# zpaq/zpaq

Hardware: AMD Instinct MI355X
Metric: compress MB/s + bit-identical ratio, -m5 over 1024x1 MiB blocks (higher is better)
Workload: dtype int32

## Files before the change

### zpaq_amd/csrc/device/pipe_kernel.h

```cpp
#pragma once
#ifndef ZPQ_LANE_VM
#define ZPQ_LANE_VM 1
#endif
#include "spec_kernel.h"

namespace zpq {

typedef __attribute__((address_space(1))) short g_i16;
typedef __attribute__((address_space(1))) unsigned short g_u16;

#ifdef ZPQ_TRACE
struct PipeTraceScope {
  unsigned long long* rec;
  __device__ __forceinline__ PipeTraceScope(const PipeArgs& a, int kernel) : rec(nullptr) {
    if (a.trace && threadIdx.x == 0) {
      rec = a.trace + 4ull * ((unsigned long long)a.trace_base + blockIdx.x);
      unsigned hw, xcc;
      asm volatile("s_getreg_b32 %0, hwreg(HW_REG_HW_ID)" : "=s"(hw));
      asm volatile("s_getreg_b32 %0, hwreg(HW_REG_XCC_ID)" : "=s"(xcc));
      rec[0] = ((unsigned long long)(unsigned)kernel << 56) | ((unsigned long long)((unsigned)a.step & 0xFFFFFFu) << 32) |
               (unsigned long long)(blockIdx.x + a.wg0);
      rec[1] = ((unsigned long long)xcc << 32) | hw;
      rec[2] = __builtin_amdgcn_s_memrealtime();
    }
// ... 1807 lines not shown
    unsigned byte = L.byte_at(0);
    uint2 w = L.bh(ri, 0);
    uint4 vj = L.p(J, 0);
    s = pipe_bh_get(w, 0);
    w0 = (int)tab[(2u * s) * G + lane]; w1 = (int)tab[(2u * s + 1u) * G + lane];
    for (unsigned k = 0; k < L.nb; ++k) {
      const unsigned kn = L.next(k);
      const unsigned byten = L.byte_at(kn);
      const uint2 wn = L.bh(ri, kn);
      const uint4 vjn = L.p(J, kn);
      do_byte(k, byte, w, wn, vj);
      byte = byten; w = wn; vj = vjn;
    }
  }
  if (store_tab)
    for (int e = 0; e < 512; e += 4)
      L.A128((unsigned)c.t0 + 4u * e) = make_uint4(tab[e * G + lane], tab[(e + 1) * G + lane], tab[(e + 2) * G + lane], tab[(e + 3) * G + lane]);
}

template <class Chain>
__device__ __forceinline__ void pipe_isse_body(const PipeArgs& a) {
  constexpr unsigned G = Chain::PIPE_G;
  __shared__ unsigned tab[512 * G];
  __shared__ PipeSquash squash;
  const int lane = threadIdx.x & 63;
  const unsigned ngroups = (a.nblocks + Chain::PIPE_G - 1u) / Chain::PIPE_G;
  const unsigned wg = blockIdx.x + a.wg0;
  const unsigned role = wg / ngroups, g = wg % ngroups;
  static_for<0, Chain::NISSE>([&](auto rc) __attribute__((always_inline)) {
    constexpr int r = decltype(rc)::value;
    if (role != (unsigned)r) return;
    constexpr int I = Chain::ISSE_COMP[r];
    PipeLane<Chain> L;
    L.open(a, g * Chain::PIPE_G + (unsigned)lane, Chain::P_LEVEL[I]);
    if (L.chunk < 0 || !pipe_any(L.nb > 0)) return;
    squash.load(a.tb, lane);
    __syncthreads();
    pipe_isse_unit<Chain, I>(L, tab, squash, lane, true, true);
  });
}

typedef uint4 __attribute__((aligned(4))) pipe_u128a4;
typedef __attribute__((address_space(1))) pipe_u128a4 g_u128a4;

template <int QL>
__device__ __forceinline__ int pipe_group_sum(int v) {
  if constexpr (QL >= 2) v += __builtin_amdgcn_update_dpp(0, v, 0xB1, 0xF, 0xF, true);
  if constexpr (QL >= 4) v += __builtin_amdgcn_update_dpp(0, v, 0x4E, 0xF, 0xF, true);
  if constexpr (QL >= 8) v += __builtin_amdgcn_update_dpp(0, v, 0x141, 0xF, 0xF, true);
  if constexpr (QL >= 16) v += __builtin_amdgcn_update_dpp(0, v, 0x140, 0xF, 0xF, true);
  return v;
}

template <class Chain, int r, class SQ>
__device__ __forceinline__ void pipe_mix_bits_unit(PipeLane<Chain>& L, unsigned q, unsigned B, const SQ& squash) {
  constexpr int I = Chain::MIX_COMP[r], QL = Chain::MIX_QL[r];
  constexpr CompK c = Chain::comp[I];
  constexpr int m = (int)c.a3, J = (int)c.a2, ci = Chain::P_CTX[I];
  constexpr int NQ = (m + 3) / 4, TAIL = m % 4, D = Chain::MIX_DEPTH, HN = D;
  static_assert(NQ <= QL && c.a5 == 255u && c.mask0 >= 255u, "MIX bit lanes need the 8 rows of a byte to be distinct");
  if (!L.nb) return;
  constexpr bool FULL = c.stride >= 4u * (unsigned)QL;
  const bool act = FULL || q < (unsigned)NQ;
  const bool tail = !FULL && TAIL != 0 && q == (unsigned)(NQ - 1);
  const unsigned qoff = 16u * (act ? q : 0u);
  bool have[4];
  int tin[4];
#pragma unroll
  for (int x = 0; x < 4; ++x) {
    const int t = (int)q * 4 + x;
    have[x] = t < m;
    tin[x] = J + (have[x] ? t : 0);
  }
  auto row_of = [&](unsigned hh, unsigned bytev) __attribute__((always_inline)) -> unsigned {
    const unsigned c8 = (1u << B) | (bytev >> (8u - B));
    return (unsigned)c.t0 + 4u * __umul24((hh + c8) & c.mask0, (unsigned)c.stride) + qoff;
  };
  auto input = [&](int x, unsigned kk) __attribute__((always_inline)) -> int {
    return (int)*(const g_i16*)((const g_u8*)&L.p(tin[x], kk) + 2u * B);
  };
  const unsigned last = L.nb - 1u;
  constexpr int W = 2 * D;
  unsigned hx[W], bx[W];
  unsigned rq[W];
  uint4 wq[W];
  int pq[W][4];
  unsigned hr[HN], hh[HN];
  uint4 hw[HN];
  auto near = [&](int sl, unsigned kk) __attribute__((always_inline)) {
    rq[sl] = row_of(hx[sl], bx[sl]);
    wq[sl] = *(g_u128a4*)(L.arena + rq[sl]);
#pragma unroll
    for (int x = 0; x < 4; ++x) pq[sl][x] = input(x, kk);
  };
#pragma unroll
  for (int sl = 0; sl < W; ++sl) {
    const unsigned kk = min((unsigned)sl, last);
    hx[sl] = L.ctx(ci, kk);
    bx[sl] = L.byte_at(kk);
  }
#pragma unroll
  for (int sl = 0; sl < D; ++sl) near(sl, min((unsigned)sl, last));
#pragma unroll
  for (int i = 0; i < HN; ++i) { hr[i] = 0xFFFFFFFFu; hh[i] = hx[0]; hw[i] = make_uint4(0u, 0u, 0u, 0u); }
  for (unsigned kb = 0; pipe_any(kb < L.nb); kb += (unsigned)W) {
#pragma unroll
// ... 31 lines not shown
        else if (act && !tail) *(g_u128a4*)(L.arena + row) = nw;
        if constexpr (TAIL != 0 && !FULL) {
          if (tail) {
            L.A32(row) = nw.x;
            if constexpr (TAIL >= 2) L.A32(row + 4u) = nw.y;
            if constexpr (TAIL >= 3) L.A32(row + 8u) = nw.z;
          }
        }
        if (q == 0) L.put_p16(I, k, B, pr);
      }
#pragma unroll
      for (int i = HN - 1; i > 0; --i) { hr[i] = hr[i - 1]; hh[i] = hh[i - 1]; hw[i] = hw[i - 1]; }
      hr[0] = row; hh[0] = hcur; hw[0] = nw;
      {
        const unsigned kw = min(k + (unsigned)W, last);
        hx[sl] = L.ctx(ci, kw);
        bx[sl] = L.byte_at(kw);
        near((sl + D) % W, min(k + (unsigned)D, last));
      }
    }
  }
}

template <class Chain>
__device__ __forceinline__ void pipe_mix_bits_body(const PipeArgs& a) {
  __shared__ PipeSquash squash;
  const int lane = threadIdx.x & 63;
  const unsigned ngroups = (a.nblocks + Chain::PIPE_G - 1u) / Chain::PIPE_G;
  const unsigned wg = blockIdx.x + a.wg0;
  squash.load(a.tb, lane);
  __syncthreads();
  static_for<0, Chain::NMIXR>([&](auto rc) __attribute__((always_inline)) {
    constexpr int r = decltype(rc)::value;
    constexpr int I = Chain::MIX_COMP[r], QL = Chain::MIX_QL[r], first = Chain::MIX_FIRST[r];
    constexpr int PPW = 64 / QL, BPW = PPW / 8;
    static_assert(QL <= 8 && BPW >= 1 && (int)Chain::PIPE_G % BPW == 0, "MIX bit lanes: a block's 8 positions share a wavefront");
    constexpr int WPG = (int)Chain::PIPE_G / BPW;
    if (wg < (unsigned)first * ngroups || wg >= (unsigned)(first + WPG) * ngroups) return;
    const unsigned wi = wg - (unsigned)first * ngroups;
    const unsigned g = wi / (unsigned)WPG, sub = wi % (unsigned)WPG;
    const unsigned pair = (unsigned)lane / QL, q = (unsigned)lane % QL, B = pair & 7u;
    PipeLane<Chain> L;
    L.open(a, pipe_opaque(g * Chain::PIPE_G + sub * BPW + (pair >> 3)), Chain::P_LEVEL[I]);
    if (L.chunk < 0 || !pipe_any(L.nb > 0)) return;
    pipe_mix_bits_unit<Chain, r>(L, q, B, squash);
  });
}

template <class Chain, int r, int NH, class SQ>
__device__ __forceinline__ void pipe_mix_unit(PipeLane<Chain>& L, unsigned q, unsigned half, const SQ& squash) {
  constexpr int I = Chain::MIX_COMP[r], QL = Chain::MIX_QL[r];
  constexpr CompK c = Chain::comp[I];
  constexpr int m = (int)c.a3, J = (int)c.a2, ci = Chain::P_CTX[I];
  constexpr int NQ = (m + 3) / 4, TAIL = m % 4, NB = 8 / NH;
  static_assert(NQ <= QL, "MIX lane group");
  constexpr bool batch = c.a5 == 255u && c.mask0 >= 255u;
  static_assert(NH == 1 || (NH == 2 && batch), "a byte is split over lane groups only when its 8 rows are distinct");
  if (!L.nb) return;
  constexpr bool FULL = c.stride >= 4u * (unsigned)QL;
  const bool act = FULL || q < (unsigned)NQ;
  const bool tail = !FULL && TAIL != 0 && q == (unsigned)(NQ - 1);
  const unsigned qoff = 16u * (act ? q : 0u);
  bool have[4];
  int tin[4];
#pragma unroll
  for (int x = 0; x < 4; ++x) {
    const int t = (int)q * 4 + x;
    have[x] = t < m;
    tin[x] = J + (have[x] ? t : 0);
  }
  auto c8_of = [&](unsigned bytev, int b) __attribute__((always_inline)) -> unsigned {
    if constexpr (NH == 1) return pipe_c8(bytev, b);
    else return ((half ? 16u : 1u) << b) | ((half ? bytev : bytev >> 4) >> (4 - b));
  };
  auto y_of = [&](unsigned bytev, int b) __attribute__((always_inline)) -> int {
    if constexpr (NH == 1) return pipe_y(bytev, b);
    else return (int)(((half ? bytev : bytev >> 4) >> (3 - b)) & 1u);
  };
  auto row_of = [&](unsigned hh, unsigned bytev, int b) __attribute__((always_inline)) -> unsigned {
    return (unsigned)c.t0 + 4u * __umul24((hh + (c8_of(bytev, b) & c.a5)) & c.mask0, (unsigned)c.stride) + qoff;
  };
  unsigned h = L.ctx(ci, 0), byte = L.byte_at(0);
  const unsigned k1 = L.next(0);
  unsigned h1 = L.ctx(ci, k1), byte1 = L.byte_at(k1);
  auto inputs = [&](int x, unsigned kk) __attribute__((always_inline)) -> uint4 {
    const uint4 v = L.p(tin[x], kk);
    const unsigned mk = have[x] ? 0xFFFFFFFFu : 0u;
    if constexpr (NH == 1) return make_uint4(v.x & mk, v.y & mk, v.z & mk, v.w & mk);
    else return make_uint4((half ? v.z : v.x) & mk, (half ? v.w : v.y) & mk, 0u, 0u);
  };
  uint4 pv[4], pv1[4];
#pragma unroll
  for (int x = 0; x < 4; ++x) { pv[x] = inputs(x, 0); pv1[x] = inputs(x, k1); }
  uint4 w[NB];
  unsigned rowc[NB];
#pragma unroll
  for (int B = 0; B < NB; ++B) rowc[B] = row_of(h, byte, B);
  if constexpr (batch) {
#pragma unroll
    for (int B = 0; B < NB; ++B) w[B] = *(g_u128a4*)(L.arena + rowc[B]);
  }
  for (unsigned k = 0; k < L.nb; ++k) {
    const unsigned k2 = min(k + 2u, L.nb - 1u);
    const unsigned h2 = L.ctx(ci, k2), byte2 = L.byte_at(k2);
    uint4 pv2[4];
#pragma unroll
    for (int x = 0; x < 4; ++x) pv2[x] = inputs(x, k2);
    unsigned rown[NB];
#pragma unroll
    for (int B = 0; B < NB; ++B) rown[B] = row_of(h1, byte1, B);
    const bool same = h1 == h;
    const bool late = !same && (((h1 - h) & c.mask0) < 256u || ((h - h1) & c.mask0) < 256u);
    uint4 wn[NB], nw[NB];
    if constexpr (batch) {
      if (!late) {
#pragma unroll
        for (int B = 0; B < NB; ++B) wn[B] = *(g_u128a4*)(L.arena + rown[B]);
      }
    }
    PipeP8 out;
#pragma unroll
    for (int B = 0; B < NB; ++B) {
      const unsigned row = rowc[B];
      if constexpr (!batch) w[B] = *(g_u128a4*)(L.arena + row);
      const int w0 = (int)w[B].x, w1 = (int)w[B].y, w2 = (int)w[B].z, w3 = (int)w[B].w;
      const int p0 = pipe_p_get(pv[0], B), p1 = pipe_p_get(pv[1], B), p2 = pipe_p_get(pv[2], B), p3 = pipe_p_get(pv[3], B);
      const int dot = __mul24(w0 >> 8, p0) + __mul24(w1 >> 8, p1) + __mul24(w2 >> 8, p2) + __mul24(w3 >> 8, p3);
      const int pr = sp_clamp2k(pipe_group_sum<QL>(dot) >> 8);
      out.set(B, pr);
      const int err = __mul24(y_of(byte, B) * 32767 - squash(pr), (int)c.a4) >> 4;
      nw[B].x = (unsigned)sp_clamp512k(w0 + ((__mul24(err, p0) + (1 << 12)) >> 13));
      nw[B].y = (unsigned)sp_clamp512k(w1 + ((__mul24(err, p1) + (1 << 12)) >> 13));
      nw[B].z = (unsigned)sp_clamp512k(w2 + ((__mul24(err, p2) + (1 << 12)) >> 13));
      nw[B].w = (unsigned)sp_clamp512k(w3 + ((__mul24(err, p3) + (1 << 12)) >> 13));
      if constexpr (FULL) *(g_u128a4*)(L.arena + row) = nw[B];
      else if (act && !tail) *(g_u128a4*)(L.arena + row) = nw[B];
      if constexpr (TAIL != 0 && !FULL) {
        if (tail) {
          L.A32(row) = nw[B].x;
          if constexpr (TAIL >= 2) L.A32(row + 4u) = nw[B].y;
          if constexpr (TAIL >= 3) L.A32(row + 8u) = nw[B].z;
        }
      }
    }
    if (q == 0) {
      if constexpr (NH == 1) L.put_p(I, k, out.get());
      else L.put_p64(I, k, half, make_uint2(out.w[0], out.w[1]));
    }
    if constexpr (batch) {
      if constexpr (NH == 2) {
        if (pipe_any(late)) pipe_stores_done();
      }
      if (late) {
#pragma unroll
        for (int B = 0; B < NB; ++B) wn[B] = *(g_u128a4*)(L.arena + rown[B]);
      }
#pragma unroll
      for (int B = 0; B < NB; ++B) {
        const bool fw = same && rown[B] == rowc[B];
        w[B].x = fw ? nw[B].x : wn[B].x; w[B].y = fw ? nw[B].y : wn[B].y;
        w[B].z = fw ? nw[B].z : wn[B].z; w[B].w = fw ? nw[B].w : wn[B].w;
      }
    }
    h = h1; byte = byte1; h1 = h2; byte1 = byte2;
#pragma unroll
    for (int B = 0; B < NB; ++B) rowc[B] = rown[B];
#pragma unroll
    for (int x = 0; x < 4; ++x) { pv[x] = pv1[x]; pv1[x] = pv2[x]; }
  }
}

struct PipeW3 { unsigned x, y, z; };
typedef __attribute__((address_space(1))) PipeW3 g_w3;

__device__ __forceinline__ int pipe_sext24(unsigned v) { return (int)(v << 8) >> 8; }
__device__ __forceinline__ void pipe_unpack4(const PipeW3& d, int& w0, int& w1, int& w2, int& w3) {
  w0 = pipe_sext24(d.x);
  w1 = pipe_sext24((d.x >> 24) | (d.y << 8));
  w2 = pipe_sext24((d.y >> 16) | (d.z << 16));
  w3 = (int)d.z >> 8;
}
__device__ __forceinline__ PipeW3 pipe_pack4(int w0, int w1, int w2, int w3) {
  PipeW3 d;
  d.x = ((unsigned)w0 & 0xFFFFFFu) | ((unsigned)w1 << 24);
  d.y = (((unsigned)w1 >> 8) & 0xFFFFu) | ((unsigned)w2 << 16);
  d.z = (((unsigned)w2 >> 16) & 0xFFu) | ((unsigned)w3 << 8);
  return d;
}

__device__ __forceinline__ constexpr unsigned pipe_mix_pstride(unsigned m) {
  const unsigned need = 12u * ((m + 3u) / 4u);
  unsigned p = 16u;
  while (p < need) p *= 2u;
  return p;
}

template <class Chain, class = void> struct PipeMixLdsRows { static constexpr int of(int) { return 0; } };
template <class Chain> struct PipeMixLdsRows<Chain, decltype((void)Chain::MIX_LDS_ROWS)> { static constexpr int of(int r) { return Chain::MIX_LDS_ROWS[r]; } };

template <class Chain, int r, int LROWS, int BPW, int NH, class SQ>
__device__ __forceinline__ void pipe_mix_packed_unit(PipeLane<Chain>& L, unsigned q, unsigned half, unsigned bl, unsigned* lds, bool stage, const SQ& squash) {
  constexpr int I = Chain::MIX_COMP[r], QL = Chain::MIX_QL[r];
  constexpr CompK c = Chain::comp[I];
  constexpr int m = (int)c.a3, J = (int)c.a2, ci = Chain::P_CTX[I];
  constexpr int NQ = (m + 3) / 4, NB = 8 / NH;
  constexpr unsigned PS = pipe_mix_pstride((unsigned)m);
  static_assert(NQ <= QL && c.a5 == 255u && c.mask0 >= 255u, "packed MIX rows: the 8 rows of a byte are distinct");
  static_assert(PS <= 4u * c.stride, "a packed row fits the padded row's place");
  static_assert(NH == 1 || NH == 2, "lane groups per block");
  if (!L.nb) return;
  const bool act = q < (unsigned)NQ;
  const unsigned qoff = 12u * (act ? q : 0u);
  bool have[4];
  int tin[4];
#pragma unroll
  for (int x = 0; x < 4; ++x) {
    const int t = (int)q * 4 + x;
    have[x] = t < m;
    tin[x] = J + (have[x] ? t : 0);
  }
  auto c8_of = [&](unsigned bytev, int b) __attribute__((always_inline)) -> unsigned {
// ... 170 lines not shown
```

### zpaq_amd/csrc/device/pipe_persist.h

```cpp
#pragma once
#include "pipe_kernel.h"

#if !defined(ZPQ_EMU)
#ifndef ZPQ_PERSIST_LDS_BYTES
#error "the generated source defines ZPQ_PERSIST_LDS_BYTES before it includes pipe_persist.h"
#endif
namespace zpq { __shared__ __attribute__((aligned(16))) unsigned char persist_lds[ZPQ_PERSIST_LDS_BYTES]; }
#endif

namespace zpq {

struct PipeRO {
  int dt[1024];
  unsigned short dt2k[256];
  PipeSquash squash;
  PipeStretch stretch;
  unsigned char ns[1024];
};

#ifdef ZPQ_EMU
#define ZPQ_PERSIST_LDS(bytes) ((unsigned char*)emu::wg_lds(bytes))
__device__ __forceinline__ unsigned pipe_prog_load(const unsigned* p) { return *(volatile const unsigned*)p; }
__device__ __forceinline__ void pipe_prog_add(unsigned* p) { *(volatile unsigned*)p = *(volatile unsigned*)p + 1u; }
__device__ __forceinline__ void pipe_flag_set(unsigned* p, unsigned v) { *(volatile unsigned*)p = v; }
// ... 198 lines not shown
      }
    } else {
      constexpr int lk = Chain::LIGHT_KIND[role], I = Chain::LIGHT_COMP[role];
      if constexpr (lk == PK_CODER) {
        if constexpr (PipeCoderFast<Chain>::value) pipe_coder_fast<Chain, (PipeAhead<Chain>::value > 0 ? PipeAhead<Chain>::value : 1)>(L, a, (unsigned*)priv, lane, c == 0);
        else pipe_coder<Chain>(L, a, ro.squash);
      } else if (pipe_any(L.nb > 0)) {
        if constexpr (lk == PK_CONS) pipe_cons<Chain, I>(L);
        else if constexpr (lk == PK_CM) {
          if constexpr (pipe_light_lds_words<Chain>(lk, I) != 0u) pipe_cm_lds<Chain, I>(L, (unsigned*)priv, ro.stretch, ro.dt, lane, c == 0);
          else pipe_cm<Chain, I>(L, ro.stretch, ro.dt);
        }
        else if constexpr (lk == PK_MATCH) pipe_match_any<Chain, I>(L, ro.stretch, ro.dt2k);
        else if constexpr (lk == PK_AVG) pipe_avg<Chain, I>(L);
        else if constexpr (lk == PK_MIX2) {
          if constexpr (pipe_light_lds_words<Chain>(lk, I) != 0u) pipe_mix2_lds<Chain, I>(L, (unsigned*)priv, ro.squash, lane, c == 0);
          else pipe_mix2<Chain, I>(L, ro.squash);
        }
        else if constexpr (lk == PK_SSE) pipe_sse<Chain, I>(L, ro.stretch, ro.dt);
        else if constexpr (lk == PK_CM_BITS) pipe_cm_bits<Chain, I>(L, B, ro.stretch, ro.dt);
        else if constexpr (lk == PK_MIX2_BITS) pipe_mix2_bits<Chain, I>(L, B, ro.squash);
        else if constexpr (lk == PK_SSE_BITS) pipe_sse_bits<Chain, I>(L, B, ro.stretch, ro.dt);
      }
    }
    pipe_reconverge();
    pipe_publish<Chain>(prog, unit, lane);
    if (a.trace) { const unsigned long long t = pipe_clock(); t_work += t - t_mark; t_mark = t; }
  }
  if (a.trace && lane == 0) {
    unsigned long long* rec = a.trace + 4ull * ((unsigned long long)g * (unsigned)Chain::PS_NSLOT + (unsigned)SLOT);
    rec[0] = t_wait; rec[1] = t_work; rec[2] = nchunks; rec[3] = ((unsigned long long)kind << 32) | ((unsigned long long)(unsigned)role << 16) | (unsigned)unit;
  }
}

template <class Chain>
__device__ __forceinline__ void pipe_persist_body(const PipeArgs& a) {
  unsigned char* const lds = ZPQ_PERSIST_LDS(Chain::PS_LDS_BYTES);
  PipeRO& ro = *(PipeRO*)lds;
  const int tid = (int)threadIdx.x, lane = tid & 63, wave = tid >> 6;
  for (int i = tid; i < 1024; i += (int)blockDim.x) ro.dt[i] = a.tb->dt[i];
  for (int i = tid; i < 256; i += (int)blockDim.x) ro.dt2k[i] = (unsigned short)a.tb->dt2k[i];
  for (int i = tid; i < 256; i += (int)blockDim.x) ((unsigned*)ro.ns)[i] = ((const unsigned*)a.tb->ns)[i];
  ro.squash.load(a.tb, tid);
  ro.stretch.load(a.tb, tid);
  if (tid == 0 && a.arrive_need) pipe_prog_add(a.ctl + 3);
  __syncthreads();
  const unsigned b = blockIdx.x, nx = a.spread ? a.spread : 1u, W = (unsigned)Chain::PS_WPG;
  const unsigned whole = a.ngroups_here - a.ngroups_here % nx;
  unsigned g, flavour;
  if (b < whole * W) { const unsigned j = b / nx; g = b % nx + nx * (j / W); flavour = j % W; }
  else { const unsigned r = b - whole * W; g = whole + r / W; flavour = r % W; }
  g += a.group0;
  if (g >= a.group0 + a.ngroups_here) return;
  const int slot = (int)flavour * Chain::PS_WAVES + wave;
  if (!pipe_arrived(a, lane)) return;
  static_for<0, Chain::PS_NSLOT>([&](auto sc) __attribute__((always_inline)) {
    constexpr int S = decltype(sc)::value;
    if constexpr (Chain::PS_KIND[S] >= 0) {
      if (slot == S) pipe_persist_unit<Chain, Chain::PS_KIND[S], Chain::PS_ROLE[S]>(a, g, lane, S);
    }
  });
}

}
```

### zpaq_amd/csrc/host/codegen.cpp

```cpp
#include "codegen.hpp"

#include <cstdio>
#include <cstdlib>
#include <cstring>
#include <map>
#include <mutex>
#include <set>
#include <sstream>
#include <algorithm>

namespace zpq {

namespace {

struct Insn { int pc, len, op; };

std::string src_expr(int k, int imm) {
  switch (k) {
    case 0: return "a";
    case 1: return "b";
    case 2: return "c";
    case 3: return "d";
    case 4: return "(unsigned)M[b & MMASK]";
    case 5: return "(unsigned)M[c & MMASK]";
// ... 568 lines not shown
  Memo m;
  m.ok = pipe_layout_compute(plan, opt, m.L, m.why);
  L = m.L; why_not = m.why;
  std::lock_guard<std::mutex> g(mu);
  if (memo.size() > 4096) memo.clear();
  memo[key] = m;
  return m.ok;
}

static bool pipe_layout_compute(const zpq_plan& plan, const PipeOptions& opt, PipeLayout& L, std::string& why_not) {
  const PlanHeader& ph = plan.hdr();
  const int n = (int)ph.n;
  if (n < 1 || n > 64) { why_not = "more than 64 components"; return false; }
  if (ph.arena_bytes >= (1ull << 32)) { why_not = "model state of 4 GiB or more per block"; return false; }
  const CompDesc* comp = plan.comps();
  L = PipeLayout();
  L.n = n;
  L.mode = opt.mode ? 1 : 0;
  L.ps_wide = opt.wide && L.mode == 1;
  if (opt.chunk >= 64 && opt.chunk <= 8192 && (opt.chunk & (opt.chunk - 1)) == 0) L.C = opt.chunk;
  if (opt.group == 8 || opt.group == 16 || opt.group == 32 || opt.group == 64) L.G = opt.group;
  enum { K_ROW = 1, K_CONS, K_CM, K_MATCH, K_AVG, K_MIX2, K_SSE, K_CODER };
  bool mix_bits_ok = true;
  L.light_bits = L.mode ? 7 : 4;
  enum { K_CM_BITS = 9, K_MIX2_BITS, K_SSE_BITS };
  auto light_unit = [&](int kind, int bits_kind, bool bits_ok, int i) {
    if (bits_ok && (L.light_bits >> (bits_kind - K_CM_BITS) & 1)) { for (int sub = 0; sub < L.G * 8 / L.light_threads(); ++sub) { L.light.push_back({bits_kind, i}); L.light_sub.push_back(sub); } }
    else { L.light.push_back({kind, i}); L.light_sub.push_back(0); }
  };
  for (int i = 0; i < n; ++i) {
    const CompDesc& c = comp[i];
    L.ctx[i] = L.row[i] = L.state[i] = -1;
    int lv = 1;
    switch (c.type) {
      case C_CONS: light_unit(K_CONS, K_CM_BITS, false, i); break;
      case C_CM: L.ctx[i] = L.nctx++; light_unit(K_CM, K_CM_BITS, c.mask0 >= 511u, i); break;
      case C_MATCH: L.ctx[i] = L.nctx++; L.state[i] = L.nstate; L.nstate += 12; light_unit(K_MATCH, K_CM_BITS, false, i); break;
      case C_ICM: L.ctx[i] = L.nctx++; L.row[i] = L.nrow++; lv = 2; L.icm.push_back(i); break;
      case C_ISSE: L.ctx[i] = L.nctx++; L.row[i] = L.nrow++; lv = std::max(2, L.level[c.a2] + 1); L.isse.push_back(i); break;
      case C_AVG: lv = std::max(L.level[c.a1], L.level[c.a2]) + 1; light_unit(K_AVG, K_CM_BITS, false, i); break;
      case C_MIX2: L.ctx[i] = L.nctx++; lv = std::max(L.level[c.a2], L.level[c.a3]) + 1;
        light_unit(K_MIX2, K_MIX2_BITS, c.a5 == 255u && c.mask0 >= 255u, i); break;
      case C_SSE: L.ctx[i] = L.nctx++; lv = L.level[c.a2] + 1; light_unit(K_SSE, K_SSE_BITS, c.mask0 >= 32u * 256u - 1u, i); break;
      case C_MIX: {
        if (c.a3 > 64) { why_not = "MIX with more than 64 inputs"; return false; }
        L.ctx[i] = L.nctx++;
        for (unsigned t = 0; t < c.a3; ++t) lv = std::max(lv, L.level[c.a2 + t] + 1);
        const int m = (int)c.a3, nq = (m + 3) / 4;
        int ql = 1;
        while (ql < nq) ql *= 2;
        if (ql > L.G) { why_not = "MIX lane group wider than the block group"; return false; }
        L.mix.push_back(i);
        L.mix_ql.push_back(ql);
        mix_bits_ok = mix_bits_ok && c.a5 == 255u && c.mask0 >= 255u && ql <= 8 && L.G * ql % 8 == 0;
        break;
      }
      default: why_not = "unknown component type"; return false;
    }
    L.level[i] = lv;
  }
  if (L.mode && mix_bits_ok && !L.mix.empty()) L.mix_bits = 1;
  for (int i = 0; i < n; ++i) if (L.row[i] >= 0) L.rows.push_back(i);
  light_unit(K_CODER, K_CM_BITS, false, n - 1);
  L.coder_level = L.level[n - 1] + 1;
  L.S = L.coder_level + 1 + L.slack;
  {
    auto kernel_of = [&](int i) { const unsigned t = comp[i].type; return t == C_ICM ? 3 : (t == C_ISSE ? 4 : (t == C_MIX ? 5 : 2)); };
    auto reads = [&](int consumer_kernel, int j) { const int pk = kernel_of(j); if (pk != consumer_kernel) L.consumes[consumer_kernel][pk] = true; };
    for (int i = 0; i < n; ++i) {
      const CompDesc& c = comp[i];
      const int k = kernel_of(i);
      if (L.ctx[i] >= 0 && c.type != C_ICM && c.type != C_ISSE) L.consumes[k][0] = true;
      if (L.row[i] >= 0) { L.consumes[1][0] = true; L.consumes[k][1] = true; }
      switch (c.type) {
        case C_ISSE: reads(k, (int)c.a2); break;
        case C_AVG: reads(k, (int)c.a1); reads(k, (int)c.a2); break;
        case C_MIX2: reads(k, (int)c.a2); reads(k, (int)c.a3); break;
        case C_SSE: reads(k, (int)c.a2); break;
        case C_MIX: for (unsigned t = 0; t < c.a3; ++t) reads(k, (int)(c.a2 + t)); break;
        default: break;
      }
    }
    reads(2, n - 1);
    L.consumes[2][0] = true;
  }
  L.hcomp_state = L.nstate; L.nstate += 8;
  L.coder_state = L.nstate; L.nstate += 4;
  const uint64_t hbytes = 4ull * (ph.hmask + 1);
  L.hcomp_h_lds = hbytes <= 8192;
  L.hcomp_lanes = 64;
  if (L.hcomp_h_lds) while (L.hcomp_lanes > 8 && hbytes * L.hcomp_lanes > 65536) L.hcomp_lanes /= 2;
  const uint64_t C = (uint64_t)L.C, S = (uint64_t)L.S, G = (uint64_t)L.G;
  uint64_t off = 0;
  L.off_ctx = off;   off += S * (uint64_t)std::max(L.nctx, 1) * C * G * 4;
  L.off_bh = off;    off += S * (uint64_t)std::max(L.nrow, 1) * C * G * 8;
  L.off_p = off;     off += S * (uint64_t)n * C * G * 16;
  L.off_state = off; off += (uint64_t)L.nstate * G * 4;
  L.group_bytes = (off + 4095) & ~4095ull;
  if (L.group_bytes >= (1ull << 32)) { why_not = "stream buffer of a block group exceeds 4 GiB"; return false; }
  L.mix_packed.assign(L.mix.size(), 0);
  static const bool packed_off = [] { const char* v = getenv("ZPAQ_AMD_MIX_PACKED"); return !(v && v[0] == '1'); }();
  for (size_t r = 0; r < L.mix.size(); ++r) {
    const CompDesc& c = comp[L.mix[r]];
    const uint32_t ps = mix_pstride(c.a3);
    if (!packed_off && !L.mix_bits && c.a5 == 255u && c.mask0 >= 255u && c.a3 >= 3u && ps <= 4u * c.stride && (ps < 4u * c.stride || c.mask0 + 1u <= 256u))
      L.mix_packed[r] = 1;
  }
  static const int rows_forced = [] { const char* v = getenv("ZPAQ_AMD_MIX_LDS_ROWS"); return v ? atoi(v) : -1; }();
  static const bool halves_wanted = [] { const char* v = getenv("ZPAQ_AMD_MIX_HALVES"); return !(v && v[0] == '0'); }();
  plan_persistent(plan, L, 0, false);
  bool halves = false;
  if (L.persist_ok && halves_wanted) {
    PipeLayout T = L;
    plan_persistent(plan, T, 0, true);
    if (T.persist_ok && T.ps_mix_nh == 2 && T.ps_wpg <= L.ps_wpg) { L = T; halves = true; }
  }
  if (L.persist_ok) {
    const int wpg0 = L.ps_wpg;
    for (int wish : {128, 64, 32}) {
      if (rows_forced >= 0 && wish != rows_forced) continue;
      PipeLayout T = L;
      plan_persistent(plan, T, wish, halves);
      bool any = false;
      for (int v : T.mix_lds_rows) any = any || v != 0;
      if (!any) break;
      if (T.persist_ok && T.ps_wpg <= wpg0) { L = T; break; }
    }
  }
  return true;
}

bool generate_pipe_source(const zpq_plan& plan, const PipeOptions& opt, std::string& source, std::string& why_not) {
  PipeLayout L;
  if (!pipe_layout(plan, opt, L, why_not)) return false;
  const PlanHeader& ph = plan.hdr();
  const int n = L.n;
  const CompDesc* comp = plan.comps();
  std::ostringstream o;
  o << "// generated by zpaq_amd codegen v" << kCodegenVersion << " (pipelined encoder) -- do not edit\n"
       "#define ZPQ_PERSIST_LDS_BYTES " << (L.persist_ok && opt.persist && opt.chunk != 2048 ? L.ps_lds_bytes : 16) << "\n"
       "#include \"pipe_persist.h\"\n"
       "namespace zpq_gen {\n"
       "struct Chain {\n";
  int nmix = 0, nsse = 0;
  std::ostringstream comps;
  for (int i = 0; i < n; ++i) {
    const CompDesc& c = comp[i];
    int slot = -1;
    if (c.type == C_MIX) slot = nmix++;
    if (c.type == C_SSE) slot = nsse++;
    comps << "    {" << c.type << "u," << c.a1 << "u," << c.a2 << "u," << c.a3 << "u," << c.a4 << "u," << c.a5 << "u, "
          << c.limit << "u," << c.mask0 << "u," << c.mask1 << "u, " << c.t0 << "ull," << c.t1 << "ull, -1," << slot << "," << c.stride << "u},\n";
  }
  auto arr = [&](const char* name, const int* v, int cnt) {
    o << "  static constexpr int " << name << "[" << std::max(cnt, 1) << "] = {";
    for (int i = 0; i < std::max(cnt, 1); ++i) o << (i ? "," : "") << (i < cnt ? v[i] : 0);
    o << "};\n";
  };
  o << "  static constexpr int N = " << n << ", NMIX = " << nmix << ", NSSE = " << nsse << ";\n"
    << "  static constexpr unsigned HMASK = " << ph.hmask << "u, MMASK = " << ph.mmask << "u;\n"
    << "  static constexpr unsigned long long OFF_RUN = " << ph.off_run << "ull;\n"
    << "  static constexpr unsigned long long OFF_H = " << ph.off_H << "ull, OFF_M = " << ph.off_M
    << "ull, OFF_R = " << ph.off_R << "ull;\n"
    << "  static constexpr zpq::CompK comp[N] = {\n" << comps.str() << "  };\n"
    << "  static constexpr unsigned PIPE_G = " << L.G << "u;\n"
    << "  static constexpr int PIPE_C = " << L.C << ", PIPE_S = " << L.S << ", PIPE_NCTX = " << std::max(L.nctx, 1)
    << ", PIPE_NROW = " << std::max(L.nrow, 1) << ";\n"
    << "  static constexpr unsigned long long PIPE_OFF_CTX = " << L.off_ctx << "ull, PIPE_OFF_BH = " << L.off_bh
    << "ull, PIPE_OFF_P = " << L.off_p << "ull, PIPE_OFF_STATE = " << L.off_state << "ull, PIPE_GROUP_BYTES = "
    << L.group_bytes << "ull;\n"
    << "  static constexpr int CODER_LEVEL = " << L.coder_level << ", CODER_STATE = " << L.coder_state
    << ", HCOMP_STATE = " << L.hcomp_state << ", HCOMP_LANES = " << L.hcomp_lanes << ";\n"
    << "  static constexpr bool HCOMP_H_LDS = " << (L.hcomp_h_lds ? "true" : "false") << ";\n";
  arr("P_LEVEL", L.level, n);
  arr("P_CTX", L.ctx, n);
  arr("P_ROW", L.row, n);
  arr("P_STATE", L.state, n);
  std::vector<int> lk, lc, mf;
  for (auto& r : L.light) { lk.push_back(r.first); lc.push_back(r.second); }
  int first = 0;
  for (int q : L.mix_ql) { mf.push_back(first); first += L.mix_waves_of(q); }
  o << "  static constexpr int PIPE_MODE = " << L.mode << ", MIX_BITS = " << L.mix_bits << ", MIX_DEPTH = " << L.depth << ";\n";
  o << "  static constexpr int NROWU = " << L.rows.size() << ", NLIGHT = " << L.light.size() << ", NICM = " << L.icm.size() << ", NISSE = " << L.isse.size()
    << ", NMIXR = " << L.mix.size() << ";\n";
  arr("LIGHT_KIND", lk.data(), (int)lk.size());
  arr("LIGHT_COMP", lc.data(), (int)lc.size());
  arr("LIGHT_SUB", L.light_sub.data(), (int)L.light_sub.size());
  o << "  static constexpr int LIGHT_THREADS = " << L.light_threads() << ", LIGHT_DEPTH = " << L.depth << ";\n";
  arr("ROW_COMP", L.rows.data(), (int)L.rows.size());
  arr("ICM_COMP", L.icm.data(), (int)L.icm.size());
  arr("ISSE_COMP", L.isse.data(), (int)L.isse.size());
  arr("MIX_COMP", L.mix.data(), (int)L.mix.size());
  arr("MIX_QL", L.mix_ql.data(), (int)L.mix_ql.size());
  arr("MIX_FIRST", mf.data(), (int)mf.size());
  arr("MIX_PACKED", L.mix_packed.data(), (int)L.mix_packed.size());
  const U8* prog = plan.blob.data() + ph.off_prog;
  if (!translate_hcomp(prog, (int)ph.prog_len, o)) { why_not = "HCOMP program too irregular to translate"; return false; }
  o << "};\n";
  if (L.persist_ok && opt.persist && opt.chunk != 2048) {
    std::vector<int> kind, role, sub, unit, ldso, dep0, ndep, du, dl, dm;
    for (size_t i = 0; i < L.ps_slots.size(); ++i) {
      const PipeLayout::Slot& sl = L.ps_slots[i];
      kind.push_back(sl.kind); role.push_back(sl.role); sub.push_back(sl.sub); unit.push_back(sl.unit); ldso.push_back(sl.lds_off);
      dep0.push_back((int)du.size()); ndep.push_back(sl.kind < 0 ? 0 : (int)L.ps_deps[i].size());
      if (sl.kind >= 0) for (const PipeLayout::Dep& d : L.ps_deps[i]) { du.push_back(d.unit); dl.push_back(d.lag); dm.push_back(d.mult); }
    }
    if (du.empty()) { du.push_back(0); dl.push_back(0); dm.push_back(0); }
    o << "struct ChainP : Chain {\n"
         "  static constexpr bool PIPE_PERSIST = true;\n"
         "  static constexpr int PS_MIX_NH = " << L.ps_mix_nh << ";\n"
         "  static constexpr bool HCOMP_M_LDS = " << (L.hcomp_m_lds ? "true" : "false") << ";\n"
         "  static constexpr int PS_AHEAD = " << L.ps_ahead << ";\n"
         "  static constexpr bool PS_ROW_RING = " << (L.ps_row_ring ? "true" : "false") << ";\n"
         "  static constexpr bool PS_CODER_FAST = " << (L.ps_coder_fast ? "true" : "false") << ", PS_SMALL = " << (L.ps_small ? "true" : "false") << ";\n"
      << (L.ps_small && !L.ps_row_halves ? "  static constexpr bool PS_ROW_HALVES = false;\n" : "")
      << (L.ps_small && !L.ps_icm_full ? "  static constexpr bool PS_ICM_FULL = false;\n" : "")
      << "";
    o <<
         "  static constexpr int PS_WAVES = " << L.ps_waves << ", PS_WPG = " << L.ps_wpg << ", PS_NSLOT = " << L.ps_slots.size()
      << ", PS_NUNIT = " << L.ps_nunit << ", PS_LDS_BYTES = " << L.ps_lds_bytes << ";\n";
    arr("PS_KIND", kind.data(), (int)kind.size());
    arr("PS_ROLE", role.data(), (int)role.size());
    arr("PS_SUB", sub.data(), (int)sub.size());
    arr("PS_UNIT", unit.data(), (int)unit.size());
    arr("PS_LDS", ldso.data(), (int)ldso.size());
    arr("PS_DEP0", dep0.data(), (int)dep0.size());
    arr("PS_NDEP", ndep.data(), (int)ndep.size());
    arr("PS_DEP_UNIT", du.data(), (int)du.size());
    arr("PS_DEP_LAG", dl.data(), (int)dl.size());
    arr("PS_DEP_MULT", dm.data(), (int)dm.size());
    arr("MIX_LDS_ROWS", L.mix_lds_rows.data(), (int)L.mix_lds_rows.size());
    o << "};\n";
  }
  o << "}  // namespace zpq_gen\n";
  if (L.persist_ok && opt.persist && opt.chunk != 2048)
    o << "extern \"C\" __global__ __launch_bounds__(" << 64 * L.ps_waves << ") void zpq_pipe_persist(zpq::PipeArgs a) {\n"
         "  zpq::pipe_persist_body<zpq_gen::ChainP>(a);\n}\n";
  else
    o << "#ifdef ZPQ_EMU\nextern \"C\" void zpq_pipe_persist(zpq::PipeArgs) {}\n#endif\n";
  o << "extern \"C\" __global__ __launch_bounds__(256) void zpq_pipe_repack(zpq::PipeArgs a) {\n"
       "  zpq::pipe_repack_body<zpq_gen::Chain>(a);\n}\n";
  const char* names[6] = {"hcomp", "rows", "light", "icm", "isse", "mix"};
  for (int k = 0; k < 6; ++k)
    o << "extern \"C\" __global__ __launch_bounds__(64) void zpq_pipe_" << names[k] << "(zpq::PipeArgs a) {\n"
         "  ZPQ_PIPE_TRACE(a, " << k << ");\n"
         "  zpq::pipe_" << names[k] << "_body<zpq_gen::Chain>(a);\n}\n";
// ... 33 lines not shown
```

### zpaq_amd/csrc/host/codegen.hpp

```cpp
#pragma once
#include <string>
#include <utility>
#include <vector>

#include "../device/plan.hpp"
#include "common.hpp"

namespace zpq {

static const int kCodegenVersion = 6;

bool generate_spec_source(const zpq_plan& plan, int waves, std::string& source, std::string& why_not, int shape = 0);
int team_threads(const zpq_plan& plan);

struct PipeOptions {
  int mode = 0;
  int chunk = 0;
  int group = 0;
  bool persist = true;
  bool wide = false;
};
static const int kPipeVariants = 4;
PipeOptions pipe_options(int variant);

struct PipeLayout {
  int n = 0;
  int C = 512;
  int G = 32;
  int S = 0;
  int nctx = 0, nrow = 0, nstate = 0;
  int level[64], ctx[64], row[64], state[64];
  int coder_level = 0, coder_state = 0, hcomp_state = 0;
  int hcomp_lanes = 64;
  bool hcomp_h_lds = false;
  bool hcomp_m_lds = false;
  std::vector<std::pair<int, int>> light;
  std::vector<int> rows, icm, isse, mix, mix_ql;
  std::vector<int> mix_packed;
  std::vector<int> mix_lds_rows;
  std::vector<int> light_sub;
  uint64_t off_ctx = 0, off_bh = 0, off_p = 0, off_state = 0, group_bytes = 0;
  bool consumes[6][6] = {};
  int slack = 3;
  int mode = 0;
  int mix_bits = 0;
  int light_bits = 4;
  int depth = 3;
  struct Slot {
    int kind = -1;
    int role = 0;
    int sub = 0;
    int unit = 0;
    int lds = 0;
    int lds_off = 0;
    float cost = 0;
    float lines = 0;
  };
  struct Dep { int unit, lag, mult; };
  bool persist_ok = false;
  std::string persist_why;
  int ps_waves = 0;
  int ps_wpg = 0;
  int ps_nunit = 0;
  int ps_lds_bytes = 0;
  bool ps_coder_fast = false;
  bool ps_row_ring = false;
  int ps_ahead = 0;
  bool ps_wide = false;
  bool ps_icm_full = false;
  bool ps_row_halves = false;
  bool ps_small = false;
  int ps_mix_nh = 1;
  std::vector<Slot> ps_slots;
  std::vector<std::vector<Dep>> ps_deps;
  int light_threads() const { return 64; }
  int mix_waves_of(int ql) const { return mix_bits ? G * ql / 8 : ql; }
  int mix_waves_per_group() const { int s = 0; for (int q : mix_ql) s += mix_waves_of(q); return s; }
  int mix_threads() const { return mix_bits ? 64 : G; }
};
bool pipe_layout(const zpq_plan& plan, const PipeOptions& opt, PipeLayout& out, std::string& why_not);
bool generate_pipe_source(const zpq_plan& plan, const PipeOptions& opt, std::string& source, std::string& why_not);

bool generate_pcomp_source(const U8* code, size_t len, int ph, int pm, std::string& source, std::string& why_not);

std::string spec_cache_key(const std::string& source);

}
```

Baseline: 391.7.

## Pack five MIX weights per lane to halve lane groups for wide mixers

Adds a per-mixer weights-per-lane setting (4 or 5). Codegen switches non-packed mixers in mode 0 to five weights per lane when that allows a smaller power-of-two lane group, cutting cross-lane reductions and wavefront count per mixer. The fifth weight is loaded, updated and forwarded with an extra scalar 32-bit access beside the 128-bit row load. It also makes the persistent-slot index wave-uniform via readfirstlane so slot dispatch can use scalar branches. A profiling script is added to report per-workgroup unit layout and estimated memory lines.

```diff
diff --git a/profiles/persist_layout.py b/profiles/persist_layout.py
--- /dev/null
+++ b/profiles/persist_layout.py
@@ -0,0 +1,66 @@
+#!/usr/bin/env python3
+import os
+import re
+import sys
+
+ROOT = os.path.dirname(os.path.dirname(os.path.abspath(__file__)))
+sys.path.insert(0, ROOT)
+
+
+def arr(src, name):
+    m = re.search(r"static constexpr int " + name + r"\[\d+\] = \{([^}]*)\}", src)
+    return [int(x) for x in m.group(1).split(",")] if m else []
+
+
+def val(src, name):
+    return int(re.search(r"\b" + name + r" = (\d+)", src).group(1))
+
+
+def main():
+    import zpaq_amd as z
+    from zpaq_amd import corpus, prebuild
+    method = sys.argv[1] if len(sys.argv) > 1 else "5"
+    kind = sys.argv[2] if len(sys.argv) > 2 else "text"
+    h = z.method_to_header(z.expand_method(method, corpus.block(kind, 1 << 20, corpus.BASE_SEED)))[0]
+    src, key = prebuild.pipe_source_and_key(h, 0)
+    comp = [[int(x) for x in re.findall(r"-?\d+", row)] for row in re.findall(r"^\s*\{(\d+u,.*?)\},$", src, re.M)]
+    G, nctx, hl = val(src, "PIPE_G"), val(src, "PIPE_NCTX"), min(val(src, "HCOMP_LANES"), val(src, "PIPE_G"))
+    W, wpg, nh = val(src, "PS_WAVES"), val(src, "PS_WPG"), val(src, "PS_MIX_NH")
+    ql, wpl = arr(src, "MIX_QL"), arr(src, "MIX_WPL") or [4] * 64
+    ctx_l, bh_l, p_l = G * 4 / 128, G * 8 / 128, G * 16 / 128
+    kinds, roles, subs = arr(src, "PS_KIND"), arr(src, "PS_ROLE"), arr(src, "PS_SUB")
+    lk, lc, mixc = arr(src, "LIGHT_KIND"), arr(src, "LIGHT_COMP"), arr(src, "MIX_COMP")
+    names = {2: "cons", 3: "cm", 4: "match", 5: "avg", 6: "mix2", 7: "sse", 8: "coder", 9: "cm/bit", 10: "mix2/bit", 11: "sse/bit"}
+
+    def slot(k, r, sub):
+        if k == 0:
+            return "hcomp", 0.0, nctx * ctx_l * hl / G
+        if k == 1:
+            return f"row{r}", 2.0 * G, ctx_l + bh_l
+        if k == 3:
+            return f"icm{r}", 0.0, bh_l + p_l
+        if k == 4:
+            return f"isse{r}", 0.0, bh_l + 2 * p_l
+        if k == 5:
+            m = comp[mixc[r]][3]
+            return f"mix{r}.{sub}({ql[r]}x{wpl[r]})", 64 / ql[r] * 8 / nh, m + ctx_l
+        t, mask0 = lk[r], comp[lc[r]][7]
+        lds = (t == 3 or (t == 6 and mask0 != 0)) and 3 <= mask0 <= 511
+        lines = 0.0 if lds else {3: 2.0 * G, 9: 16.0, 4: 3.0 * G, 6: 8.0 * G if mask0 else 0.0, 10: 64.0, 7: 8.0 * G, 11: 64.0}.get(t, 0.0)
+        sl = (p_l if t == 8 else p_l + ctx_l) + (2 * p_l if t in (5, 6, 10) else (p_l if t in (7, 11) else 0.0))
+        if t >= 9:
+            sl *= 64 / (G * 8)
+        return f"{names.get(t, '?')}{lc[r]}" + (f".{sub}" if t >= 9 else ""), lines, sl
+
+    print(f"method {method} {kind}: cache key {key}; {wpg} workgroups x {W} wavefronts per group of {G} blocks, MIX lane groups per block {nh}")
+    tot_t = tot_s = used = 0
+    for b in range(wpg):
+        items = [slot(kinds[b * W + w], roles[b * W + w], subs[b * W + w]) for w in range(W) if kinds[b * W + w] >= 0]
+        t, s = sum(i[1] for i in items), sum(i[2] for i in items)
+        tot_t += t; tot_s += s; used += len(items)
+        print(f"  workgroup {b}: {len(items)} units, {t:6.0f} table + {s:5.1f} stream = {t + s:6.1f} lines per byte:  " + " ".join(i[0] for i in items))
+    print(f"  group: {used} unit wavefronts of {wpg * W} slots, {tot_t:.0f} table + {tot_s:.1f} stream = {tot_t + tot_s:.1f} lines per input byte")
+
+
+if __name__ == "__main__":
+    main()
diff --git a/zpaq_amd/csrc/device/pipe_kernel.h b/zpaq_amd/csrc/device/pipe_kernel.h
--- a/zpaq_amd/csrc/device/pipe_kernel.h
+++ b/zpaq_amd/csrc/device/pipe_kernel.h
@@ -1883,6 +1883,9 @@
   return v;
 }
 
+template <class Chain, class = void> struct PipeMixWpl { static constexpr int of(int) { return 4; } };
+template <class Chain> struct PipeMixWpl<Chain, decltype((void)Chain::MIX_WPL)> { static constexpr int of(int r) { return Chain::MIX_WPL[r]; } };
+
 template <class Chain, int r, class SQ>
 __device__ __forceinline__ void pipe_mix_bits_unit(PipeLane<Chain>& L, unsigned q, unsigned B, const SQ& squash) {
   constexpr int I = Chain::MIX_COMP[r], QL = Chain::MIX_QL[r];
@@ -2020,20 +2023,22 @@
   constexpr int I = Chain::MIX_COMP[r], QL = Chain::MIX_QL[r];
   constexpr CompK c = Chain::comp[I];
   constexpr int m = (int)c.a3, J = (int)c.a2, ci = Chain::P_CTX[I];
-  constexpr int NQ = (m + 3) / 4, TAIL = m % 4, NB = 8 / NH;
-  static_assert(NQ <= QL, "MIX lane group");
+  constexpr int WPL = PipeMixWpl<Chain>::of(r);
+  constexpr int NQ = (m + WPL - 1) / WPL, TAIL = m % WPL, NB = 8 / NH;
+  static_assert((WPL == 4 || WPL == 5) && NQ <= QL, "MIX lane group");
   constexpr bool batch = c.a5 == 255u && c.mask0 >= 255u;
   static_assert(NH == 1 || (NH == 2 && batch), "a byte is split over lane groups only when its 8 rows are distinct");
   if (!L.nb) return;
-  constexpr bool FULL = c.stride >= 4u * (unsigned)QL;
+  constexpr bool FULL = c.stride >= (unsigned)(WPL * QL);
+  static_assert(WPL == 4 || FULL, "five weights per lane: the lane group's slots lie inside the padded row");
   const bool act = FULL || q < (unsigned)NQ;
   const bool tail = !FULL && TAIL != 0 && q == (unsigned)(NQ - 1);
-  const unsigned qoff = 16u * (act ? q : 0u);
-  bool have[4];
-  int tin[4];
-#pragma unroll
-  for (int x = 0; x < 4; ++x) {
-    const int t = (int)q * 4 + x;
+  const unsigned qoff = 4u * (unsigned)WPL * (act ? q : 0u);
+  bool have[WPL];
+  int tin[WPL];
+#pragma unroll
+  for (int x = 0; x < WPL; ++x) {
+    const int t = (int)q * WPL + x;
     have[x] = t < m;
     tin[x] = J + (have[x] ? t : 0);
   }
@@ -2057,43 +2062,56 @@
     if constexpr (NH == 1) return make_uint4(v.x & mk, v.y & mk, v.z & mk, v.w & mk);
     else return make_uint4((half ? v.z : v.x) & mk, (half ? v.w : v.y) & mk, 0u, 0u);
   };
-  uint4 pv[4], pv1[4];
-#pragma unroll
-  for (int x = 0; x < 4; ++x) { pv[x] = inputs(x, 0); pv1[x] = inputs(x, k1); }
+  uint4 pv[WPL], pv1[WPL];
+#pragma unroll
+  for (int x = 0; x < WPL; ++x) { pv[x] = inputs(x, 0); pv1[x] = inputs(x, k1); }
   uint4 w[NB];
+  unsigned w4[NB];
   unsigned rowc[NB];
 #pragma unroll
   for (int B = 0; B < NB; ++B) rowc[B] = row_of(h, byte, B);
   if constexpr (batch) {
 #pragma unroll
-    for (int B = 0; B < NB; ++B) w[B] = *(g_u128a4*)(L.arena + rowc[B]);
+    for (int B = 0; B < NB; ++B) {
+      w[B] = *(g_u128a4*)(L.arena + rowc[B]);
+      if constexpr (WPL == 5) w4[B] = L.A32(rowc[B] + 16u);
+    }
   }
   for (unsigned k = 0; k < L.nb; ++k) {
     const unsigned k2 = min(k + 2u, L.nb - 1u);
     const unsigned h2 = L.ctx(ci, k2), byte2 = L.byte_at(k2);
-    uint4 pv2[4];
-#pragma unroll
-    for (int x = 0; x < 4; ++x) pv2[x] = inputs(x, k2);
+    uint4 pv2[WPL];
+#pragma unroll
+    for (int x = 0; x < WPL; ++x) pv2[x] = inputs(x, k2);
     unsigned rown[NB];
 #pragma unroll
     for (int B = 0; B < NB; ++B) rown[B] = row_of(h1, byte1, B);
     const bool same = h1 == h;
     const bool late = !same && (((h1 - h) & c.mask0) < 256u || ((h - h1) & c.mask0) < 256u);
     uint4 wn[NB], nw[NB];
+    unsigned wn4[NB], nw4[NB];
     if constexpr (batch) {
       if (!late) {
 #pragma unroll
-        for (int B = 0; B < NB; ++B) wn[B] = *(g_u128a4*)(L.arena + rown[B]);
+        for (int B = 0; B < NB; ++B) {
+          wn[B] = *(g_u128a4*)(L.arena + rown[B]);
+          if constexpr (WPL == 5) wn4[B] = L.A32(rown[B] + 16u);
+        }
       }
     }
     PipeP8 out;
 #pragma unroll
     for (int B = 0; B < NB; ++B) {
       const unsigned row = rowc[B];
-      if constexpr (!batch) w[B] = *(g_u128a4*)(L.arena + row);
+      if constexpr (!batch) {
+        w[B] = *(g_u128a4*)(L.arena + row);
+        if constexpr (WPL == 5) w4[B] = L.A32(row + 16u);
+      }
       const int w0 = (int)w[B].x, w1 = (int)w[B].y, w2 = (int)w[B].z, w3 = (int)w[B].w;
       const int p0 = pipe_p_get(pv[0], B), p1 = pipe_p_get(pv[1], B), p2 = pipe_p_get(pv[2], B), p3 = pipe_p_get(pv[3], B);
-      const int dot = __mul24(w0 >> 8, p0) + __mul24(w1 >> 8, p1) + __mul24(w2 >> 8, p2) + __mul24(w3 >> 8, p3);
+      int dot = __mul24(w0 >> 8, p0) + __mul24(w1 >> 8, p1) + __mul24(w2 >> 8, p2) + __mul24(w3 >> 8, p3);
+      int p4 = 0;
+      if constexpr (WPL == 5) { p4 = pipe_p_get(pv[4], B); dot += __mul24((int)w4[B] >> 8, p4); }
       const int pr = sp_clamp2k(pipe_group_sum<QL>(dot) >> 8);
       out.set(B, pr);
       const int err = __mul24(y_of(byte, B) * 32767 - squash(pr), (int)c.a4) >> 4;
@@ -2101,6 +2119,10 @@
       nw[B].y = (unsigned)sp_clamp512k(w1 + ((__mul24(err, p1) + (1 << 12)) >> 13));
       nw[B].z = (unsigned)sp_clamp512k(w2 + ((__mul24(err, p2) + (1 << 12)) >> 13));
       nw[B].w = (unsigned)sp_clamp512k(w3 + ((__mul24(err, p3) + (1 << 12)) >> 13));
+      if constexpr (WPL == 5) {
+        nw4[B] = (unsigned)sp_clamp512k((int)w4[B] + ((__mul24(err, p4) + (1 << 12)) >> 13));
+        L.A32(row + 16u) = nw4[B];
+      }
       if constexpr (FULL) *(g_u128a4*)(L.arena + row) = nw[B];
       else if (act && !tail) *(g_u128a4*)(L.arena + row) = nw[B];
       if constexpr (TAIL != 0 && !FULL) {
@@ -2121,20 +2143,24 @@
       }
       if (late) {
 #pragma unroll
-        for (int B = 0; B < NB; ++B) wn[B] = *(g_u128a4*)(L.arena + rown[B]);
+        for (int B = 0; B < NB; ++B) {
+          wn[B] = *(g_u128a4*)(L.arena + rown[B]);
+          if constexpr (WPL == 5) wn4[B] = L.A32(rown[B] + 16u);
+        }
       }
 #pragma unroll
       for (int B = 0; B < NB; ++B) {
         const bool fw = same && rown[B] == rowc[B];
         w[B].x = fw ? nw[B].x : wn[B].x; w[B].y = fw ? nw[B].y : wn[B].y;
         w[B].z = fw ? nw[B].z : wn[B].z; w[B].w = fw ? nw[B].w : wn[B].w;
+        if constexpr (WPL == 5) w4[B] = fw ? nw4[B] : wn4[B];
       }
     }
     h = h1; byte = byte1; h1 = h2; byte1 = byte2;
 #pragma unroll
     for (int B = 0; B < NB; ++B) rowc[B] = rown[B];
 #pragma unroll
-    for (int x = 0; x < 4; ++x) { pv[x] = pv1[x]; pv1[x] = pv2[x]; }
+    for (int x = 0; x < WPL; ++x) { pv[x] = pv1[x]; pv1[x] = pv2[x]; }
   }
 }
 
diff --git a/zpaq_amd/csrc/device/pipe_persist.h b/zpaq_amd/csrc/device/pipe_persist.h
--- a/zpaq_amd/csrc/device/pipe_persist.h
+++ b/zpaq_amd/csrc/device/pipe_persist.h
@@ -274,7 +274,11 @@
   else { const unsigned r = b - whole * W; g = whole + r / W; flavour = r % W; }
   g += a.group0;
   if (g >= a.group0 + a.ngroups_here) return;
+#ifdef ZPQ_EMU
   const int slot = (int)flavour * Chain::PS_WAVES + wave;
+#else
+  const int slot = __builtin_amdgcn_readfirstlane((int)flavour * Chain::PS_WAVES + wave);
+#endif
   if (!pipe_arrived(a, lane)) return;
   static_for<0, Chain::PS_NSLOT>([&](auto sc) __attribute__((always_inline)) {
     constexpr int S = decltype(sc)::value;
diff --git a/zpaq_amd/csrc/host/codegen.cpp b/zpaq_amd/csrc/host/codegen.cpp
--- a/zpaq_amd/csrc/host/codegen.cpp
+++ b/zpaq_amd/csrc/host/codegen.cpp
@@ -644,6 +644,7 @@
         if (ql > L.G) { why_not = "MIX lane group wider than the block group"; return false; }
         L.mix.push_back(i);
         L.mix_ql.push_back(ql);
+        L.mix_wpl.push_back(4);
         mix_bits_ok = mix_bits_ok && c.a5 == 255u && c.mask0 >= 255u && ql <= 8 && L.G * ql % 8 == 0;
         break;
       }
@@ -698,6 +699,15 @@
     if (!packed_off && !L.mix_bits && c.a5 == 255u && c.mask0 >= 255u && c.a3 >= 3u && ps <= 4u * c.stride && (ps < 4u * c.stride || c.mask0 + 1u <= 256u))
       L.mix_packed[r] = 1;
   }
+  if (L.mode == 0)
+    for (size_t r = 0; r < L.mix.size(); ++r) {
+      if (L.mix_packed[r]) continue;
+      const CompDesc& c = comp[L.mix[r]];
+      const int m = (int)c.a3;
+      int q5 = 1;
+      while (q5 * 5 < m) q5 *= 2;
+      if (q5 * 5 < L.mix_ql[r] * 4 && c.stride >= (uint32_t)(q5 * 5)) { L.mix_ql[r] = q5; L.mix_wpl[r] = 5; }
+    }
   static const int rows_forced = [] { const char* v = getenv("ZPAQ_AMD_MIX_LDS_ROWS"); return v ? atoi(v) : -1; }();
   static const bool halves_wanted = [] { const char* v = getenv("ZPAQ_AMD_MIX_HALVES"); return !(v && v[0] == '0'); }();
   plan_persistent(plan, L, 0, false);
@@ -784,6 +794,7 @@
   arr("ISSE_COMP", L.isse.data(), (int)L.isse.size());
   arr("MIX_COMP", L.mix.data(), (int)L.mix.size());
   arr("MIX_QL", L.mix_ql.data(), (int)L.mix_ql.size());
+  if (std::any_of(L.mix_wpl.begin(), L.mix_wpl.end(), [](int w) { return w != 4; })) arr("MIX_WPL", L.mix_wpl.data(), (int)L.mix_wpl.size());
   arr("MIX_FIRST", mf.data(), (int)mf.size());
   arr("MIX_PACKED", L.mix_packed.data(), (int)L.mix_packed.size());
   const U8* prog = plan.blob.data() + ph.off_prog;
diff --git a/zpaq_amd/csrc/host/codegen.hpp b/zpaq_amd/csrc/host/codegen.hpp
--- a/zpaq_amd/csrc/host/codegen.hpp
+++ b/zpaq_amd/csrc/host/codegen.hpp
@@ -36,6 +36,7 @@
   bool hcomp_m_lds = false;
   std::vector<std::pair<int, int>> light;
   std::vector<int> rows, icm, isse, mix, mix_ql;
+  std::vector<int> mix_wpl;
   std::vector<int> mix_packed;
   std::vector<int> mix_lds_rows;
   std::vector<int> light_sub;
```

New measurement: 367.6. 0.938x the previous value.
